# TurakhiaLab/WEPP

Hardware: AMD Instinct MI355X
Metric: reads placed/sec on SARS-CoV-2 MAT (~16M nodes) (higher is better)
Workload: dtype int32

## Files before the change

__graft_entry__.py:

```python
import os
import subprocess
import sys

ROOT = os.path.dirname(os.path.abspath(__file__))
if ROOT not in sys.path:
    sys.path.insert(0, ROOT)
sys.path.insert(0, os.path.join(ROOT, "tests"))


def build():
    subprocess.check_call(["make", "-C", os.path.join(ROOT, "wepp_amd", "csrc"), "-j4"])
    csrc = os.path.join(ROOT, "wepp_amd", "csrc")
    variant = os.path.join(ROOT, "variants", "win64", "libwepp_place.so")
    newest = max(os.path.getmtime(os.path.join(csrc, f)) for f in os.listdir(csrc) if f.endswith((".hip", ".cpp", ".hpp")))
    if not os.path.exists(variant) or os.path.getmtime(variant) < newest:
        subprocess.check_call(["bash", os.path.join(ROOT, "tools", "build_variant.sh"), "win64", "-DWEPP_WIN_SIZE=64", "-DWEPP_WIN_STRIDE=32"],
                              stdout=subprocess.DEVNULL)
    import oracle_bridge
    oracle_bridge.build()
    import wepp_amd


def smoke():
    import numpy as np
    import oracle_bridge
    import wepp_amd as w

    g = w.generate_tree(7, 3000, genome_len=2000, p_ambiguous=0.01, p_masked_node=0.002, root_mutations=2)
    reads = g.reads(8, 256, read_len=150, amplicon_len=400, amplicon_step=300, p_substitution=0.004, p_n=0.01,
                    p_iupac=0.1)
    mat = w.Mat(g.tree, device=0)
    res = mat.place_batch(reads)
    want = oracle_bridge.OracleTree(g.tree).place_batch(reads, nthreads=4)
    assert (res.score == want["score"]).all(), "parsimony scores differ from the oracle"
    assert (res.best_bfs_j == want["best_j"]).all(), "placement nodes differ from the oracle"
    assert (res.num_best == want["num_best"]).all(), "num_best differs from the oracle"
    assert (res.has_unique == want["has_unique"]).all(), "has_unique differs from the oracle"
    mat.close()
    print("smoke ok: %d reads placed on a %d-node MAT, bit-exact vs oracle" % (reads.n_reads, g.tree.n_nodes))

# ... 6 lines not shown
```

wepp_amd/csrc/capi.cpp:

```cpp
#include <hip/hip_runtime.h>

#include <algorithm>
#include <atomic>
#include <functional>
#include <cstdio>
#include <cstdlib>
#include <chrono>
#include <cstring>
#include <new>
#include <string>
#include <thread>
#include <vector>

#include "handle.hpp"
#include "host_pool.hpp"

namespace {

std::atomic<uint32_t> g_handles_alive{0};

void release(wepp_mat* h) {
    if (!h) return;
    g_handles_alive.fetch_sub(1, std::memory_order_relaxed);
    (void)hipSetDevice(h->device);
// ... 178 lines not shown
                a_nest.insert(a_nest.end(), st.ix_nest.begin(), st.ix_nest.end());
                a_nrec.insert(a_nrec.end(), st.nrec.begin(), st.nrec.end());
                a_pre.insert(a_pre.end(), st.rq_pre.begin(), st.rq_pre.end());
                a_suf.insert(a_suf.end(), st.rq_suf.begin(), st.rq_suf.end());
                a_dst.insert(a_dst.end(), st.rq_dst.begin(), st.rq_dst.end());
                a_sp.insert(a_sp.end(), st.sp.begin(), st.sp.end());
                h->wc_nodes += st.n;
                h->wc_count++;
            }
        DevWalk arena{};
        auto dev_array = [&](auto*& out, size_t count, const auto& front) -> int {
            using T = std::remove_cv_t<std::remove_reference_t<decltype(front[0])>>;
            void* p = nullptr;
            const size_t bytes = std::max<size_t>(count * sizeof(T), 16);
            hipError_t e2 = hipMalloc(&p, bytes);
            if (e2 != hipSuccess) return set_error(WEPP_ENOMEM, std::string("hipMalloc: ") + hipGetErrorString(e2));
            h->allocs.push_back(p);
            h->stats.device_bytes += bytes;
            if (!front.empty()) HIP_TRY(hipMemcpy(p, front.data(), front.size() * sizeof(T), hipMemcpyHostToDevice));
            out = (T*)p;
            return WEPP_OK;
        };
        IxHead* g_head; IxEnt* g_ent; uint8_t *g_nest, *g_sp; NodeRec* g_nrec; SegNode *g_pre, *g_suf, *g_dst;
#define ARR(ptr, count, front) if ((rc = dev_array(ptr, count, front)) != WEPP_OK) { release(h); return rc; }
        ARR(g_head, tot_head, a_head) ARR(g_ent, tot_ent, a_ent) ARR(g_nest, tot_head, a_nest) ARR(g_sp, tot_sp, a_sp)
        ARR(g_nrec, tot_n, a_nrec) ARR(g_pre, tot_n, a_pre) ARR(g_suf, tot_n, a_suf) ARR(g_dst, tot_dst, a_dst)
#undef ARR
        arena.ix_head = g_head; arena.ix_ent = g_ent; arena.ix_nest = g_nest; arena.sp = g_sp;
        arena.nrec = g_nrec; arena.rq_pre = g_pre; arena.rq_suf = g_suf; arena.rq_dst = g_dst;
        {
            size_t o_n = wc_n, o_ent = wc_ent, o_head = wc_head, o_sp = wc_sp, o_dst = wc_dst;
            for (size_t i = 0; i < f.streams.size(); i++) {
                const Stream& st = f.streams[i];
                WcInfo& wi = info[n_wc + i];
                wi.n = st.n;
                wi.rq_blocks = st.rq_blocks;
                wi.last_ent = (uint32_t)(o_ent + st.ix_ent.size() - 1);
                wi.has_pre = st.ix_pre.empty() ? 0u : st.ix_pre[0];
                wi.node_off = (uint32_t)o_n; wi.head_off = (uint32_t)o_head; wi.nest_off = (uint32_t)o_head; wi.dst_off = (uint32_t)o_dst;
                wi.sp_off = o_sp;
                wi.tau = st.tau;
                wi.whole = st.whole;
                wi.whole_bfs = f.rank2bfs[st.whole.rank < f.N ? st.whole.rank : 0u];
#define CP(dst, off, vec) if (!vec.empty()) HIP_TRY(hipMemcpy(dst + off, vec.data(), vec.size() * sizeof(vec[0]), hipMemcpyHostToDevice));
                CP(g_head, o_head, st.ix_head) CP(g_ent, o_ent, st.ix_ent) CP(g_nest, o_head, st.ix_nest) CP(g_sp, o_sp, st.sp)
                CP(g_nrec, o_n, st.nrec) CP(g_pre, o_n, st.rq_pre) CP(g_suf, o_n, st.rq_suf) CP(g_dst, o_dst, st.rq_dst)
#undef CP
                if (o_ent) HIP_TRY(launch_rebase_index(g_head + o_head, (uint32_t)st.ix_head.size(), g_ent + o_ent, (uint32_t)st.ix_ent.size(), (uint32_t)o_ent, nullptr));
                DevWalk& dw = h->walks[i];
                dw.n = st.n; dw.rq_blocks = st.rq_blocks; dw.last_ent = wi.last_ent; dw.has_pre = wi.has_pre; dw.whole = st.whole;
                dw.ix_head = g_head + o_head; dw.ix_ent = g_ent; dw.ix_nest = g_nest + o_head; dw.nrec = g_nrec + o_n;
                dw.rq_pre = g_pre + o_n; dw.rq_suf = g_suf + o_n; dw.rq_dst = g_dst + o_dst; dw.sp = g_sp + o_sp;
                o_n += st.n; o_ent += st.ix_ent.size(); o_head += st.ix_head.size(); o_sp += st.sp.size(); o_dst += st.rq_dst.size();
            }
            HIP_TRY(hipDeviceSynchronize());
        }
        d.tw_base = (uint32_t)n_wc;
        {
            std::vector<int64_t> s_nkey;
            std::vector<uint32_t> s_nstat, s_node0, s_eoff, s_evw, s_cpo, s_cpw;
            std::vector<uint8_t> s_meta, s_lb;
            std::vector<BlkSum> s_sum;
            struct Off { size_t nkey, node0, eoff, sum, ev, cpo, cpw; };
            std::vector<Off> offs;
            for (const auto& wc : f.wcrowns)
                for (const Stream& st : wc) {
                    offs.push_back(Off{s_nkey.size(), s_node0.size(), s_eoff.size(), s_sum.size(), s_evw.size(), s_cpo.size(), s_cpw.size()});
                    s_nkey.insert(s_nkey.end(), st.nkey.begin(), st.nkey.end());
                    s_nstat.insert(s_nstat.end(), st.nstat.begin(), st.nstat.end());
                    s_node0.insert(s_node0.end(), st.blk_node0.begin(), st.blk_node0.end());
                    s_eoff.insert(s_eoff.end(), st.blk_eoff.begin(), st.blk_eoff.end());
// ... 15 lines not shown
            std::vector<DevStream> ws(f.wcrowns.size() * WC_MAX, DevStream{});
            size_t k = 0;
            for (size_t w = 0; w < f.wcrowns.size(); w++)
                for (size_t i = 0; i < f.wcrowns[w].size(); i++, k++) {
                    const Stream& st = f.wcrowns[w][i];
                    DevStream& ds = ws[w * WC_MAX + i];
                    ds.n = st.n; ds.NB = st.NB; ds.cp_stride = st.cp_stride; ds.ncp = (uint32_t)st.cp_off.size() - 1;
                    ds.eager = 1u; ds.tier = WC_SLOT; ds.e_pad = (uint32_t)st.E;
                    ds.nkey = d_nkey + offs[k].nkey; ds.nstat = d_nstat + offs[k].nkey;
                    ds.blk_node0 = d_node0 + offs[k].node0; ds.blk_eoff = d_eoff + offs[k].eoff; ds.blk_sum = d_sum + offs[k].sum;
                    ds.ev_word = d_evw + offs[k].ev; ds.ev_meta = d_meta + offs[k].ev; ds.ev_lb = d_lb + offs[k].ev;
                    ds.cp_off = d_cpo + offs[k].cpo; ds.cp_word = d_cpw + offs[k].cpw;
                }
            UP(d.wc_streams, ws)
        }
        UP(d.wc_info, info)
        d.wc_windows = (uint32_t)f.wcrowns.size();
        h->stats.n_window_crowns = h->wc_count;
        h->stats.window_crown_nodes = h->wc_nodes;
        h->walks.resize(MAX_STREAMS, DevWalk{});
        h->walks[WC_SLOT] = arena;
    }
    UP(d.walks, h->walks)
    d.seed_sig = nullptr;
    d.seed_stride = d.seed_chunks = d.seed_row_words = 0;
    if (!f.seed_sig.empty()) {
        UP(d.seed_sig, f.seed_sig)
        d.seed_stride = f.seed_stride;
        d.seed_chunks = f.seed_chunks;
        d.seed_row_words = f.seed_row_words;
    }
    h->use_seeds = h->tun.seed ? 1 : 0;
    h->stats.seed_chunks = d.seed_chunks;
    h->stats.seed_chunk_blocks = d.seed_stride;
    h->stats.seed_sig_bytes = (uint64_t)f.seed_sig.size() * 4;
    h->stats.window_size = WIN_SIZE;
    h->stats.window_stride = WIN_STRIDE;
    h->stats.window_uncovered_positions = f.max_pos + 1 > MAX_WINDOWS * WIN_STRIDE ? f.max_pos + 1 - MAX_WINDOWS * WIN_STRIDE : 0;
#undef UP
    {
        const bool walk_on = h->tun.walk;
        h->walk_ok = 1;
        for (const Stream& st : f.streams)
            if ((uint64_t)st.n >= (1ull << (32 - WALK_DELTA_BITS))) h->walk_ok = 0;
        h->use_walk = (walk_on && h->walk_ok) ? 1 : 0;
    }
// ... 1398 lines not shown
```

wepp_amd/csrc/device_mat.hpp:

```cpp
#pragma once
#include <hip/hip_runtime.h>
#include <stdint.h>

#include "flatmat.hpp"

namespace wepp {

constexpr int32_t SCORE_INF_DEV = SCORE_INF;
constexpr uint32_t NS_CNT_MASK_DEV = NS_CNT_MASK;
constexpr uint32_t NS_LEAF_DEV = NS_LEAF, NS_MASKED_DEV = NS_MASKED, NS_ELIG0_DEV = NS_ELIG0, NS_ROOT_DEV = NS_ROOT;
constexpr uint32_t EV_OFF_MASK_DEV = EV_OFF_MASK;
constexpr uint32_t W_EXIT_DEV = W_EXIT, W_LEAF_DEV = W_LEAF, W_PAD_DEV = W_PAD;
constexpr uint32_t WEPP_FLAG_HAS_UNIQUE_DEV = WEPP_FLAG_HAS_UNIQUE;

constexpr uint32_t EV_TAIL_PAD = 128, SUM_TAIL_PAD = 4;
struct DevStream {
    uint32_t n, NB, cp_stride, ncp;
    uint32_t eager;
    uint32_t tier;
    uint32_t e_pad;
    const int64_t* nkey;
    const uint32_t* nstat;
    const uint32_t* blk_node0;
    const uint32_t* blk_eoff;
    const BlkSum* blk_sum;
    const uint32_t* ev_word;
    const uint8_t* ev_meta;
// ... 4 lines not shown
};

struct DevWalk {
    uint32_t n, rq_blocks, last_ent, has_pre;
    SegNode whole;
    const IxHead* ix_head;
    const IxEnt* ix_ent;
    const uint8_t* ix_nest;
    const NodeRec* nrec;
    const SegNode* rq_pre;
    const SegNode* rq_suf;
    const SegNode* rq_dst;
    const uint8_t* sp;
};

struct WcInfo {
    uint32_t n, rq_blocks, last_ent, has_pre;
    uint32_t node_off, head_off, nest_off, dst_off;
    unsigned long long sp_off;
    int32_t tau;
    uint32_t whole_bfs;
    SegNode whole;
};

struct DevMAT {
    uint32_t N, bm_words, max_pos, n_streams;
    uint32_t n_windows;
    uint32_t walk_eager_nodes;
    int32_t root_base;
    int32_t tau[MAX_STREAMS];
    const uint32_t* node_woff;
    const uint32_t* words;
    const uint32_t* nstat;
    const uint32_t* rank2dfs;
    const uint32_t* dfs2bfs;
    const uint32_t* rank2bfs;
    const uint32_t* bfs2dfs;
    const uint32_t* parent_dfs;
    const uint8_t* maxnest;
    const DevWalk* walks;
    const WcInfo* wc_info;
    const DevStream* wc_streams;
    uint32_t wc_windows;
    uint32_t tw_base;
    uint32_t win_n[MAX_WINDOWS];
    const uint32_t* seed_sig;
    uint32_t seed_stride, seed_chunks, seed_row_words;
};
constexpr uint32_t WIN_MIN_ENTRIES = 32;

constexpr uint32_t MAX_PLANS = 128;
constexpr uint32_t PLAN_WALK8 = 0, PLAN_WALK16 = 1, PLAN_SWEEP = 2, PLAN_WALKC8 = 3, PLAN_WALKC16 = 4, PLAN_WIN = 5, PLAN_SEED = 6;
constexpr uint32_t PLAN_WIN_BASE = PLAN_WIN * MAX_STREAMS;
constexpr uint32_t PLAN_SEED_ID = PLAN_WIN_BASE + MAX_WINDOWS;
static_assert(PLAN_SEED_ID < MAX_PLANS, "plan ids");
__host__ __device__ inline uint32_t plan_id(uint32_t cls, uint32_t idx) { return cls == PLAN_SEED ? PLAN_SEED_ID : cls * MAX_STREAMS + idx; }
__host__ __device__ inline uint32_t plan_class(uint32_t id) { return id == PLAN_SEED_ID ? PLAN_SEED : id >= PLAN_WIN_BASE ? PLAN_WIN : id / MAX_STREAMS; }
__host__ __device__ inline uint32_t plan_index(uint32_t id) { return id == PLAN_SEED_ID ? 0u : id >= PLAN_WIN_BASE ? id - PLAN_WIN_BASE : id % MAX_STREAMS; }
constexpr uint32_t SEED_MIN_HARD = 3;
constexpr uint32_t SEED_MIN_STREAM_NODES = 65536;
constexpr uint32_t SEED_MAX_ENTRIES = 4096;
#ifndef WEPP_SEED_THREADS
#define WEPP_SEED_THREADS 512
#endif
constexpr uint32_t SEED_THREADS = WEPP_SEED_THREADS;
constexpr uint32_t SEED_HEAVY_LEVEL_MIN = 256, SEED_HEAVY_PARTS = 32, SEED_HEAVY_CAP = 128;
constexpr uint32_t SEED_MAX_HARD = 255;
// ... 90 lines not shown
constexpr uint32_t ROUTE_BLOCKS = WEPP_ROUTE_BLOCKS;
constexpr uint32_t ROUTE_THREADS = 1024;

struct RouteDirect {
    uint32_t* wlist[2];
    uint32_t* clist[2];
    uint32_t* jobs[2];
    uint32_t* job_first;
    uint32_t* wwlist;
    uint32_t* best_bfs_j;
    int32_t* score;
    uint32_t* num_best;
    uint32_t* flags;
    unsigned long long* work_counter;
    uint32_t cand_min;
    uint32_t ww_max_small, ww_max_big;
};
hipError_t launch_route(const DevMAT& m, const uint32_t* d_read_off, const uint32_t* d_read_word, uint32_t n_reads,
                        int use_crowns, uint32_t walk_max_events, uint32_t job_events, uint32_t stack8, uint32_t stack16,
                        uint32_t seed_min_hard, uint32_t seed_min_nodes,
                        uint32_t* job_n, uint8_t* tier_of, int32_t* root_score, uint32_t* blk_counts,
                        uint32_t* tier_info, uint32_t* slot_in_blk, uint32_t* tier_info_next, uint32_t* wsid, const RouteDirect& direct,
                        hipStream_t stream);
hipError_t launch_rebase_index(IxHead* heads, uint32_t n_heads, IxEnt* ents, uint32_t n_ents, uint32_t ent_off, hipStream_t stream);
uint32_t seed_lds_bytes(const DevMAT& m, uint32_t ent_cap);
hipError_t seed_set_max_lds(uint32_t bytes);
size_t seed_heavy_bytes();
hipError_t launch_seed(const DevMAT& m, const DevStream& full, const uint32_t* list, uint32_t n_list, uint32_t ent_cap,
                       const uint32_t* d_read_off, const uint32_t* d_read_word, const int32_t* root_score,
                       uint32_t* best_bfs_j, int32_t* score, uint32_t* num_best, uint32_t* flags,
                       unsigned long long* work_counter, void* heavy_table, hipStream_t stream);
constexpr uint32_t SORT_KEY_BITS = 21;
constexpr uint32_t SORT_MIN_READS = 4096;
constexpr uint32_t WALK_SORT_KEY_BITS = SORT_KEY_BITS + 4;
constexpr uint32_t WALK_SORT_MIN_READS = 32768;
static_assert(MAX_STREAMS <= 16, "stream index in the walks' sort key");
hipError_t launch_first_pos(const uint32_t* list, uint32_t n, const uint32_t* d_read_off, const uint32_t* d_read_word,
                            uint32_t* keys, hipStream_t stream);
hipError_t launch_walk_keys(const uint32_t* list, uint32_t n, const uint8_t* tier_of, const uint32_t* d_read_off,
                            const uint32_t* d_read_word, uint32_t* keys, hipStream_t stream);
hipError_t sort_reads_temp_bytes(uint32_t n, size_t* bytes);
hipError_t launch_sort_reads(const uint32_t* keys_in, uint32_t* keys_out, const uint32_t* vals_in, uint32_t* vals_out,
                             uint32_t n, void* temp, size_t temp_bytes, hipStream_t stream, uint32_t key_bits = SORT_KEY_BITS);
hipError_t launch_scatter(const uint8_t* tier_of, const uint32_t* slot_in_blk, uint32_t n_reads, const uint32_t* blk_counts,
                          uint32_t* tier_info, uint32_t* list, bool skip_plain_walks, hipStream_t stream);
hipError_t launch_sweep(const DevMAT& m, const DevStream& st, const uint32_t* d_read_off,
// ... 85 lines not shown
```

wepp_amd/csrc/flat_debug.cpp:

```cpp
#include <cstdlib>
#include <cstring>
#include <new>
#include <string>

#include "../../include/wepp_place.h"
#include "errors.hpp"
#include "flatmat.hpp"

extern "C" uint64_t wepp_debug_flatten_count(void) { return wepp::flatten_count(); }

extern "C" int wepp_flat_create(const wepp_tree_desc* tree, wepp_flat_t** out) {
    if (!tree || !out) return wepp::set_error(WEPP_EINVAL, "null argument");
    *out = nullptr;
    wepp_flat* h = new (std::nothrow) wepp_flat();
    if (!h) return wepp::set_error(WEPP_ENOMEM, "out of host memory");
    std::string err;
    int rc;
    try {
        rc = wepp::flatten_tree(*tree, h->f, err);
    } catch (const std::bad_alloc&) {
        delete h;
        return wepp::set_error(WEPP_ENOMEM, "out of host memory while flattening the tree");
    }
    if (rc != WEPP_OK) { delete h; return wepp::set_error(rc, err); }
    *out = h;
    return WEPP_OK;
}

extern "C" int wepp_flat_get(const wepp_flat_t* flat, const char* name, const void** data, uint64_t* count,
                             uint32_t* elem_bytes) {
    if (!flat || !name || !data || !count || !elem_bytes) return wepp::set_error(WEPP_EINVAL, "null argument");
    const wepp::FlatMAT& f = flat->f;
// ... 99 lines not shown
```

wepp_amd/csrc/route_kernels.hip:

```cpp
#include <hip/hip_runtime.h>
#include <stdint.h>

#include <algorithm>

#include "device_mat.hpp"
#include "place_dev.hpp"

namespace wepp {

#ifdef WEPP_ROUTE_STATS
__device__ unsigned long long g_route_stats[16];
#define ROUTE_STAMP(i) do { __builtin_amdgcn_sched_barrier(0); __builtin_amdgcn_s_waitcnt(0); { const unsigned long long now_ = __builtin_amdgcn_s_memtime(); \
    if (blockIdx.x == 0 && threadIdx.x == 0) g_route_stats[i] += now_ - last_; last_ = now_; } __builtin_amdgcn_sched_barrier(0); } while (0)
#define ROUTE_STAMP_NW(i) do { __builtin_amdgcn_sched_barrier(0); { const unsigned long long now_ = __builtin_amdgcn_s_memtime(); \
    if (blockIdx.x == 0 && threadIdx.x == 0) g_route_stats[i] += now_ - last_; last_ = now_; } __builtin_amdgcn_sched_barrier(0); } while (0)
#else
#define ROUTE_STAMP(i)
#define ROUTE_STAMP_NW(i)
#endif

__global__ __launch_bounds__(ROUTE_THREADS) void k_route(DevMAT m, const uint32_t* __restrict__ read_off,
                                                          const uint32_t* __restrict__ read_word, uint32_t n_reads,
                                                          int use_crowns, uint32_t walk_max_events, uint32_t job_events,
                                                          uint32_t stack8, uint32_t stack16,
                                                          uint32_t seed_min_hard, uint32_t seed_min_nodes,
                                                          uint32_t* __restrict__ job_n, uint8_t* __restrict__ tier_of,
                                                          int32_t* __restrict__ root_score,
                                                          uint32_t* __restrict__ blk_counts,
                                                          uint32_t* __restrict__ tier_info,
                                                          uint32_t* __restrict__ slot_in_blk,
                                                          uint32_t* __restrict__ tier_info_next,
                                                          uint32_t* __restrict__ wsid, RouteDirect direct) {
#ifdef WEPP_ROUTE_STATS
    unsigned long long last_ = __builtin_amdgcn_s_memtime();
#endif
    __shared__ uint32_t cnt[MAX_PLANS], mx[MAX_PLANS], jobs_of[2 * MAX_STREAMS], open_of[4], events_of[2], resolved_of[1];
    constexpr uint32_t RT_MAX = MAX_WINDOWS * WC_MAX + MAX_STREAMS;
    __shared__ int32_t wc_tau[RT_MAX], rt_wbase[RT_MAX];
    __shared__ uint32_t wc_n[RT_MAX], rt_head[RT_MAX], rt_nest[RT_MAX], rt_wbfs[RT_MAX], rt_wcnt[RT_MAX];
    for (uint32_t i = threadIdx.x; i < m.tw_base + m.n_streams && i < RT_MAX; i += blockDim.x) {
        const WcInfo q = m.wc_info[i];
        wc_tau[i] = q.tau; wc_n[i] = q.n; rt_head[i] = q.head_off; rt_nest[i] = q.nest_off;
        rt_wbase[i] = q.whole.base; rt_wbfs[i] = q.whole_bfs; rt_wcnt[i] = (q.whole.cnt << 1) | (q.whole.hu ? 1u : 0u);
    }
    constexpr uint32_t TT_MAX = 64, WT_D = 8;
    __shared__ uint8_t t_tab[TT_MAX], sid_tab[MAX_WINDOWS * WT_D];
    __shared__ uint32_t tab_ok[1];
    if (threadIdx.x == 0) tab_ok[0] = (m.n_streams >= 2 && m.tau[m.n_streams - 2] < (int32_t)TT_MAX && m.tau[0] >= 0) ? 1u : 0u;
    __syncthreads();
    if (threadIdx.x < TT_MAX) {
        uint32_t t = m.n_streams - 1;
        for (uint32_t i = 0; i + 1 < m.n_streams; i++)
            if ((int32_t)threadIdx.x <= m.tau[i]) { t = i; break; }
        t_tab[threadIdx.x] = (uint8_t)t;
    }
    if (threadIdx.x < m.wc_windows * WT_D && threadIdx.x < MAX_WINDOWS * WT_D) {
        const uint32_t wi = threadIdx.x / WT_D, d = threadIdx.x % WT_D;
        uint32_t pick = 0xFFu;
        for (uint32_t i = 0; i < WC_MAX; i++) {
            const int32_t tau = wc_tau[wi * WC_MAX + i];
            if (!wc_n[wi * WC_MAX + i]) break;
            if (tau != 0x7FFFFFFF && (tau < m.root_base || tau >= m.root_base + (int32_t)(WT_D - 1))) atomicAnd(&tab_ok[0], 0u);
            if (pick == 0xFFu && m.root_base + (int32_t)d <= tau) pick = i;
        }
        sid_tab[threadIdx.x] = (uint8_t)pick;
    }
    __shared__ uint32_t wl_count[2], wl_base[2], cj_count[2], cl_count[2], cj_base[2], cl_base[2], c_ok[2], ww_count[2], ww_base[2], w16_to_wave[1], ww_cand[2];
    if (threadIdx.x < 2) { cj_count[threadIdx.x] = 0; cl_count[threadIdx.x] = 0; }
    if (threadIdx.x == 0) ww_count[0] = ww_count[1] = ww_cand[0] = ww_cand[1] = 0;
    if (threadIdx.x == 0) resolved_of[0] = 0;
    if (threadIdx.x < 2) wl_count[threadIdx.x] = 0;
    if (blockIdx.x == 0 && threadIdx.x < TI_WORDS) tier_info_next[threadIdx.x] = 0;
    if (threadIdx.x < MAX_PLANS) { cnt[threadIdx.x] = 0; mx[threadIdx.x] = 0; }
    if (threadIdx.x < 4) open_of[threadIdx.x] = 0;
    if (threadIdx.x < 2) events_of[threadIdx.x] = 0;
    if (threadIdx.x < 2 * MAX_STREAMS) jobs_of[threadIdx.x] = 0;
    __syncthreads();
    ROUTE_STAMP(0);
    const uint32_t per = (n_reads + gridDim.x - 1) / gridDim.x;
    const uint32_t lo = blockIdx.x * per, hi = min(n_reads, lo + per);
    const IxHead* __restrict__ ar_head = m.walks[WC_SLOT].ix_head;
    const uint8_t* __restrict__ ar_nest = m.walks[WC_SLOT].ix_nest;
    const uint32_t root_w0 = m.node_woff[0], root_w1 = m.node_woff[1];
    const bool use_tabs = tab_ok[0] != 0;
    const uint32_t lane = threadIdx.x & 63;
    const unsigned long long lt_mask = (1ull << lane) - 1ull;
    for (uint32_t rbase = lo; rbase < hi; rbase += 4 * blockDim.x) {
      const uint32_t r0 = rbase + threadIdx.x;
      uint32_t so4[4], k4[4], fw[4][2];
      uint32_t app4[4] = {0, 0, 0, 0}, aslot4[4] = {0, 0, 0, 0};
      uint32_t cj4[4] = {0, 0, 0, 0}, cjs4[4] = {0, 0, 0, 0}, cls4[4] = {0, 0, 0, 0}, cnj4[4] = {0, 0, 0, 0};
      uint32_t ww4[4] = {0, 0, 0, 0};
#pragma unroll
      for (uint32_t u = 0; u < 4; u++) {
          const uint32_t r = r0 + u * blockDim.x;
          so4[u] = r < hi ? read_off[r] : 0u;
          k4[u] = r < hi ? read_off[r + 1] - so4[u] : 0u;
      }
#pragma unroll
      for (uint32_t u = 0; u < 4; u++)
#pragma unroll
          for (uint32_t j = 0; j < 2; j++) fw[u][j] = k4[u] > j ? read_word[so4[u] + j] : 0u;
      ROUTE_STAMP(1);
      int c4[4] = {0, 0, 0, 0};
      uint32_t nh4[4] = {0, 0, 0, 0}, t4[4] = {0, 0, 0, 0}, sid4[4] = {NONE, NONE, NONE, NONE}, wi4[4] = {0, 0, 0, 0}, inwin4[4] = {0, 0, 0, 0};
      uint32_t pre_nest[4][2] = {{0, 0}, {0, 0}, {0, 0}, {0, 0}}, pre_o0[4][2] = {{0, 0}, {0, 0}, {0, 0}, {0, 0}}, pre_o1[4][2] = {{0, 0}, {0, 0}, {0, 0}, {0, 0}};
#pragma unroll
      for (uint32_t u = 0; u < 4; u++) {
        const uint32_t r = r0 + u * blockDim.x;
        const uint32_t k = k4[u], so = so4[u];
        if (r < hi) {
            int c = 0;
            auto count = [&](uint32_t sw) { if (!rw_missing(sw)) c += ((rw_mut(sw) & rw_ref(sw)) == 0) ? 1 : 0; };
            if (k > 0) count(fw[u][0]);
            if (k > 1) count(fw[u][1]);
            for (uint32_t j = 2; j < k; j++) count(read_word[so + j]);
            nh4[u] = (uint32_t)c;
            for (uint32_t w = root_w0; w < root_w1; w++) {
                const uint32_t tw = m.words[w];
                uint32_t sw = NONE;
                if (k <= 2) {
                    if (k > 0 && w_pos(fw[u][0]) == w_pos(tw)) sw = fw[u][0];
                    if (k > 1 && w_pos(fw[u][1]) == w_pos(tw)) sw = fw[u][1];
                } else sw = find_entry(read_word, so, k, w_pos(tw));
                if (sw != NONE) c += enter_delta(tw, sw);
            }
            c4[u] = c;
            ROUTE_STAMP_NW(2);
            const int theta = m.root_base + c + (int)k;
// ... 10 lines not shown
                const uint32_t p_lo = w_pos(fw[u][0]), p_hi = w_pos(k > 2 ? read_word[so + k - 1] : k == 2 ? fw[u][1] : fw[u][0]);
                const uint32_t wi = p_lo / WIN_STRIDE;
                wi4[u] = wi;
                inwin4[u] = p_hi < wi * WIN_STRIDE + WIN_SIZE ? 1u : 0u;
                if (inwin4[u] && wi < m.wc_windows) {
                    const int rs = m.root_base + c;
                    if (use_tabs) {
                        const uint32_t i = sid_tab[wi * WT_D + (uint32_t)min(max(c, 0), (int)WT_D - 1)];
                        if (i != 0xFFu && wc_n[wi * WC_MAX + i] < wc_n[m.tw_base + t]) sid4[u] = wi * WC_MAX + i;
                    } else
                        for (uint32_t i = 0; i < WC_MAX; i++) {
                            const uint32_t qn = wc_n[wi * WC_MAX + i];
                            if (!qn) break;
                            if (rs <= wc_tau[wi * WC_MAX + i]) { if (qn < wc_n[m.tw_base + t]) sid4[u] = wi * WC_MAX + i; break; }
                        }
                }
            }
            ROUTE_STAMP_NW(4);
            if (walk_max_events && k <= WALK16_K) {
                const uint32_t tab = sid4[u] != NONE ? sid4[u] : m.tw_base + t;
#pragma unroll
                for (uint32_t j = 0; j < 2; j++) {
                    const uint32_t p = w_pos(fw[u][j]);
                    if (j < k && p <= m.max_pos) {
                        pre_nest[u][j] = (uint32_t)ar_nest[rt_nest[tab] + p];
                        pre_o0[u][j] = ar_head[rt_head[tab] + p].off;
                        pre_o1[u][j] = ar_head[rt_head[tab] + p + 1].off;
                    }
                }
            }
        }
      }
      ROUTE_STAMP(5);
#pragma unroll
      for (uint32_t u = 0; u < 4; u++) {
        const uint32_t r = r0 + u * blockDim.x;
        const bool valid = r < hi;
        uint32_t t_id = 0, append = 0;
        bool resolved = false;
        const uint32_t k = k4[u];
        if (valid) {
        const uint32_t so = so4[u];
        const int c = c4[u];
        const uint32_t n_hard = nh4[u];
        uint32_t t = t4[u];
        const uint32_t sid = sid4[u], wi = wi4[u];
        const bool in_win = inwin4[u] != 0;
        const uint32_t pre_tab = sid != NONE ? sid : m.tw_base + t;
        uint32_t cls = PLAN_SWEEP;
        auto classify = [&](uint32_t tab, uint32_t& nj_out, uint32_t& open_out, uint32_t& ev_out) -> uint32_t {
            const IxHead* ix_head = ar_head + rt_head[tab];
            const uint8_t* ix_nest = ar_nest + rt_nest[tab];
            uint32_t open_max = 0, events = 0, longest = 0;
            for (uint32_t j = 0; j < k; j++) {
                const uint32_t p = w_pos(j == 0 ? fw[u][0] : j == 1 ? fw[u][1] : read_word[so + j]);
                if (p <= m.max_pos) {
                    uint32_t nest, o0, o1;
                    if (j < 2 && tab == pre_tab) { nest = j ? pre_nest[u][1] : pre_nest[u][0]; o0 = j ? pre_o0[u][1] : pre_o0[u][0]; o1 = j ? pre_o1[u][1] : pre_o1[u][0]; }
                    else { nest = (uint32_t)ix_nest[p]; o0 = ix_head[p].off; o1 = ix_head[p + 1].off; }
                    open_max += nest;
                    const uint32_t len = o1 - o0 - 1u;
                    events += len;
                    longest = max(longest, len);
                }
            }
            open_out = open_max;
            ev_out = events;
            nj_out = 0;
            if (events <= walk_max_events) {
                if (k <= WALK8_K && open_max <= stack8) return PLAN_WALK8;
                if (open_max <= stack16) return PLAN_WALK16;
                return PLAN_SWEEP;
            }
            if (open_max > stack16) return PLAN_SWEEP;
            const uint32_t small = (k <= WALK8_K && open_max <= stack8) ? 1u : 0u;
            const uint32_t je = small ? (job_events & 0xFFFFu) : (job_events >> 16);
            nj_out = min((events + je - 1) / je, longest);
            return small ? PLAN_WALKC8 : PLAN_WALKC16;
        };
        if (walk_max_events && k <= WALK16_K) {
            uint32_t nj = 0, open_max = 0, events = 0;
            if (sid != NONE) {
                cls = classify(sid, nj, open_max, events);
                if (cls != PLAN_SWEEP) { wsid[r] = sid; t = WC_SLOT; }
// ... 74 lines not shown
            }
            if (listed) slot_in_blk[r] = slot;
        }
        {
            const unsigned long long rm = __ballot(resolved);
            if (rm && lane == (uint32_t)__builtin_ctzll(rm)) atomicAdd(&resolved_of[0], (uint32_t)__popcll(rm));
        }
        if (direct.wlist[0]) {
#pragma unroll
            for (uint32_t cc = 0; cc < 2; cc++) {
                const unsigned long long mk = __ballot(append == cc + 1);
                if (!mk) continue;
                const int first = __builtin_ctzll(mk);
                uint32_t base = 0;
                if ((int)lane == first) base = atomicAdd(&wl_count[cc], (uint32_t)__popcll(mk));
                base = (uint32_t)__builtin_amdgcn_readlane((int)base, first);
                if (append == cc + 1) { app4[u] = cc + 1; aslot4[u] = base + (uint32_t)__popcll(mk & lt_mask); }
            }
        }
        ROUTE_STAMP(6);
      }
      if (direct.wlist[0]) {
          __syncthreads();
          if (threadIdx.x < 2) {
              const uint32_t cc = threadIdx.x;
              const bool to_wave = cc == 1 && direct.wwlist && wl_count[1] && wl_count[1] <= WALK16_TO_WAVE_MAX;
              if (cc == 1) w16_to_wave[0] = to_wave ? 1u : 0u;
              if (to_wave) {
                  wl_base[1] = atomicAdd(&tier_info[TI_WWCUR], wl_count[1]);
                  atomicAdd(&tier_info[TI_W16WAVE], wl_count[1]);
              } else
                  wl_base[cc] = wl_count[cc] ? atomicAdd(&tier_info[TI_WCUR + cc], wl_count[cc]) : 0u;
              wl_count[cc] = 0;
              c_ok[cc] = 0;
              if (cl_count[cc] && direct.jobs[0]) {
                  cj_base[cc] = atomicAdd(&tier_info[TI_JCUR + cc], cj_count[cc]);
                  cl_base[cc] = atomicAdd(&tier_info[TI_CCUR + cc], cl_count[cc]);
                  if (cj_base[cc] + cj_count[cc] > BLIND_JOB_CAP || cl_base[cc] + cl_count[cc] > BLIND_CHUNKED_READS) tier_info[TI_JOVER + cc] = 1u;
                  else c_ok[cc] = 1;
              }
              cj_count[cc] = 0;
              cl_count[cc] = 0;
              if (cc == 0) {
                  for (uint32_t b = 0; b < 2; b++) {
                      const uint32_t n = min(ww_count[b], b ? direct.ww_max_big : direct.ww_max_small);
                      ww_base[b] = n ? atomicAdd(&tier_info[TI_WWCUR + b], n) : 0u;
                      ww_count[b] = 0;
                  }
              }
          }
          __syncthreads();
#pragma unroll
          for (uint32_t u = 0; u < 4; u++) {
              const uint32_t r = r0 + u * blockDim.x;
              if (app4[u]) (app4[u] == 1 ? direct.wlist[0] : w16_to_wave[0] ? direct.wwlist : direct.wlist[1])[wl_base[app4[u] - 1] + aslot4[u]] = r;
              if (ww4[u]) {
                  const uint32_t big = ww4[u] & 1u, at = ww_base[big] + (ww4[u] >> 1) - 1u;
                  direct.wwlist[big ? n_reads - 1u - at : at] = r;
              }
              if (cj4[u] && c_ok[cj4[u] - 1]) {
                  const uint32_t cc = cj4[u] - 1, j0 = cj_base[cc] + cjs4[u];
                  (cc ? direct.clist[1] : direct.clist[0])[cl_base[cc] + cls4[u]] = r;
                  direct.job_first[r] = j0;
                  uint32_t* jt = cc ? direct.jobs[1] : direct.jobs[0];
                  for (uint32_t c2 = 0; c2 < cnj4[u]; c2++) jt[j0 + c2] = r;
              }
          }
          __syncthreads();
      }
      ROUTE_STAMP(7);
    }
    __syncthreads();
// ... 9 lines not shown
    if (threadIdx.x < 2 && events_of[threadIdx.x]) atomicAdd(&tier_info[TI_EVENTS + threadIdx.x], (events_of[threadIdx.x] + 63) >> 6);
    if (threadIdx.x < 2 && ww_cand[threadIdx.x]) atomicAdd(&tier_info[TI_WWCAND + threadIdx.x], ww_cand[threadIdx.x]);
    if (threadIdx.x == 0 && resolved_of[0]) {
        atomicAdd(&tier_info[TI_RESOLVED], resolved_of[0]);
        if (direct.work_counter) atomicAdd(direct.work_counter + WALK_COUNTERS + (blockIdx.x & (WALK_COUNTERS - 1)), 48ull * resolved_of[0]);
    }
    ROUTE_STAMP(8);
#ifdef WEPP_ROUTE_STATS
    if (blockIdx.x == 0 && threadIdx.x == 0) g_route_stats[9] += 1;
#endif
}
#ifdef WEPP_ROUTE_STATS
extern "C" int wepp_debug_route_stats(unsigned long long* out16) {
    return (int)hipMemcpyFromSymbol(out16, HIP_SYMBOL(g_route_stats), sizeof(g_route_stats));
}
#endif

__global__ void k_rebase_index(IxHead* __restrict__ heads, uint32_t n_heads, IxEnt* __restrict__ ents, uint32_t n_ents, uint32_t ent_off) {
    const uint32_t i = blockIdx.x * blockDim.x + threadIdx.x;
    if (i < n_heads) heads[i].off += ent_off;
    if (i < n_ents && ents[i].up != IX_NONE) ents[i].up += ent_off;
}

__global__ __launch_bounds__(ROUTE_THREADS) void k_scatter(const uint8_t* __restrict__ tier_of,
                                                            const uint32_t* __restrict__ slot_in_blk, uint32_t n_reads,
                                                            const uint32_t* __restrict__ blk_counts,
                                                            uint32_t* __restrict__ tier_info,
                                                            uint32_t* __restrict__ list, int skip_plain_walks) {
    __shared__ uint32_t base[MAX_PLANS], before[MAX_PLANS];
    if (threadIdx.x < MAX_PLANS) before[threadIdx.x] = 0;
    __syncthreads();
    {
        const uint32_t t = threadIdx.x & (MAX_PLANS - 1), c0 = threadIdx.x / MAX_PLANS;
        uint32_t acc = 0;
        for (uint32_t b = c0; b < blockIdx.x; b += blockDim.x / MAX_PLANS) acc += blk_counts[b * MAX_PLANS + t];
        if (acc) atomicAdd(&before[t], acc);
    }
    __syncthreads();
    if (threadIdx.x < MAX_PLANS) {
        const uint32_t t = threadIdx.x;
        uint32_t off = 0;
        for (uint32_t i = 0; i < t; i++) off += tier_info[TI_COUNT + i];
        base[t] = off + before[t];
        if (blockIdx.x == 0) {
            tier_info[TI_OFF + t] = off;
            if (t == MAX_PLANS - 1) tier_info[TI_OFF + MAX_PLANS] = off + tier_info[TI_COUNT + t];
// ... 28 lines not shown
}

__global__ void k_walk_keys(const uint32_t* __restrict__ list, uint32_t n, const uint8_t* __restrict__ tier_of,
                            const uint32_t* __restrict__ read_off, const uint32_t* __restrict__ read_word,
                            uint32_t* __restrict__ keys) {
    const uint32_t i = blockIdx.x * blockDim.x + threadIdx.x;
    if (i >= n) return;
    const uint32_t r = list[i], so = read_off[r];
    const uint32_t first = (read_off[r + 1] > so) ? w_pos(read_word[so]) + 1u : 0u;
    keys[i] = (plan_index(tier_of[r]) << SORT_KEY_BITS) | first;
}

hipError_t launch_route(const DevMAT& m, const uint32_t* d_read_off, const uint32_t* d_read_word, uint32_t n_reads,
                        int use_crowns, uint32_t walk_max_events, uint32_t job_events, uint32_t stack8, uint32_t stack16,
                        uint32_t seed_min_hard, uint32_t seed_min_nodes, uint32_t* job_n, uint8_t* tier_of,
                        int32_t* root_score, uint32_t* blk_counts, uint32_t* tier_info, uint32_t* slot_in_blk,
                        uint32_t* tier_info_next, uint32_t* wsid, const RouteDirect& direct, hipStream_t stream) {
    hipLaunchKernelGGL(k_route, dim3(ROUTE_BLOCKS), dim3(ROUTE_THREADS), 0, stream, m, d_read_off, d_read_word,
                       n_reads, use_crowns, walk_max_events, job_events, std::min(stack8, WALK8_STACK), std::min(stack16, WALK16_STACK),
                       seed_min_hard, seed_min_nodes, job_n, tier_of, root_score, blk_counts, tier_info, slot_in_blk, tier_info_next, wsid, direct);
    return hipGetLastError();
}

hipError_t launch_rebase_index(IxHead* heads, uint32_t n_heads, IxEnt* ents, uint32_t n_ents, uint32_t ent_off, hipStream_t stream) {
    const uint32_t n = std::max(n_heads, n_ents);
    if (!n) return hipSuccess;
    hipLaunchKernelGGL(k_rebase_index, dim3((n + 255) / 256), dim3(256), 0, stream, heads, n_heads, ents, n_ents, ent_off);
    return hipGetLastError();
}

hipError_t launch_first_pos(const uint32_t* list, uint32_t n, const uint32_t* d_read_off, const uint32_t* d_read_word,
                            uint32_t* keys, hipStream_t stream) {
    if (n == 0) return hipSuccess;
    hipLaunchKernelGGL(k_first_pos, dim3((n + 255) / 256), dim3(256), 0, stream, list, n, d_read_off, d_read_word, keys);
    return hipGetLastError();
}

hipError_t launch_walk_keys(const uint32_t* list, uint32_t n, const uint8_t* tier_of, const uint32_t* d_read_off,
                            const uint32_t* d_read_word, uint32_t* keys, hipStream_t stream) {
    if (n == 0) return hipSuccess;
    hipLaunchKernelGGL(k_walk_keys, dim3((n + 255) / 256), dim3(256), 0, stream, list, n, tier_of, d_read_off, d_read_word, keys);
    return hipGetLastError();
}

hipError_t launch_scatter(const uint8_t* tier_of, const uint32_t* slot_in_blk, uint32_t n_reads, const uint32_t* blk_counts,
                          uint32_t* tier_info, uint32_t* list, bool skip_plain_walks, hipStream_t stream) {
    hipLaunchKernelGGL(k_scatter, dim3(ROUTE_BLOCKS), dim3(ROUTE_THREADS), 0, stream, tier_of, slot_in_blk, n_reads,
                       blk_counts, tier_info, list, skip_plain_walks ? 1 : 0);
    return hipGetLastError();
}

}
```

Baseline: 10.91 billion.

## Precompute packed per-position route words and route tables once at load

Adds a load-time pass that packs each index position's event-list length and nesting depth into one dword, so the route classifier does one load per position instead of a byte plus two IxHead offsets. The per-block shared-memory routing tables, previously rebuilt at the start of every k_route block, are now built once by a one-block kernel and bulk-copied into LDS. The end-of-batch atomic reservations are also spread across a wave's lanes instead of being serialized in two threads. It costs an extra device array the size of the index heads and falls back to the old two-offset path when a length saturates.

```diff
diff --git a/__graft_entry__.py b/__graft_entry__.py
--- a/__graft_entry__.py
+++ b/__graft_entry__.py
@@ -11,11 +11,11 @@
 def build():
     subprocess.check_call(["make", "-C", os.path.join(ROOT, "wepp_amd", "csrc"), "-j4"])
     csrc = os.path.join(ROOT, "wepp_amd", "csrc")
-    variant = os.path.join(ROOT, "variants", "win64", "libwepp_place.so")
     newest = max(os.path.getmtime(os.path.join(csrc, f)) for f in os.listdir(csrc) if f.endswith((".hip", ".cpp", ".hpp")))
-    if not os.path.exists(variant) or os.path.getmtime(variant) < newest:
-        subprocess.check_call(["bash", os.path.join(ROOT, "tools", "build_variant.sh"), "win64", "-DWEPP_WIN_SIZE=64", "-DWEPP_WIN_STRIDE=32"],
-                              stdout=subprocess.DEVNULL)
+    for name, flags in (("win64", ["-DWEPP_WIN_SIZE=64", "-DWEPP_WIN_STRIDE=32"]), ("rtlen3", ["-DWEPP_RT_LEN_BITS=3"])):
+        variant = os.path.join(ROOT, "variants", name, "libwepp_place.so")
+        if not os.path.exists(variant) or os.path.getmtime(variant) < newest:
+            subprocess.check_call(["bash", os.path.join(ROOT, "tools", "build_variant.sh"), name, *flags], stdout=subprocess.DEVNULL)
     import oracle_bridge
     oracle_bridge.build()
     import wepp_amd
diff --git a/wepp_amd/csrc/capi.cpp b/wepp_amd/csrc/capi.cpp
--- a/wepp_amd/csrc/capi.cpp
+++ b/wepp_amd/csrc/capi.cpp
@@ -224,12 +224,20 @@
             return WEPP_OK;
         };
         IxHead* g_head; IxEnt* g_ent; uint8_t *g_nest, *g_sp; NodeRec* g_nrec; SegNode *g_pre, *g_suf, *g_dst;
+        uint32_t* g_rtpos;
 #define ARR(ptr, count, front) if ((rc = dev_array(ptr, count, front)) != WEPP_OK) { release(h); return rc; }
         ARR(g_head, tot_head, a_head) ARR(g_ent, tot_ent, a_ent) ARR(g_nest, tot_head, a_nest) ARR(g_sp, tot_sp, a_sp)
         ARR(g_nrec, tot_n, a_nrec) ARR(g_pre, tot_n, a_pre) ARR(g_suf, tot_n, a_suf) ARR(g_dst, tot_dst, a_dst)
+        ARR(g_rtpos, tot_head, std::vector<uint32_t>())
 #undef ARR
         arena.ix_head = g_head; arena.ix_ent = g_ent; arena.ix_nest = g_nest; arena.sp = g_sp;
         arena.nrec = g_nrec; arena.rq_pre = g_pre; arena.rq_suf = g_suf; arena.rq_dst = g_dst;
+        d.rt_pos = g_rtpos;
+        for (size_t w = 0; w < f.wcrowns.size(); w++)
+            for (size_t i = 0; i < f.wcrowns[w].size(); i++) {
+                const WcInfo& wi = info[w * WC_MAX + i];
+                HIP_TRY(launch_route_pos(g_head + wi.head_off, g_nest + wi.nest_off, (uint32_t)f.wcrowns[w][i].ix_head.size(), g_rtpos + wi.head_off, nullptr));
+            }
         {
             size_t o_n = wc_n, o_ent = wc_ent, o_head = wc_head, o_sp = wc_sp, o_dst = wc_dst;
             for (size_t i = 0; i < f.streams.size(); i++) {
@@ -249,6 +257,7 @@
                 CP(g_nrec, o_n, st.nrec) CP(g_pre, o_n, st.rq_pre) CP(g_suf, o_n, st.rq_suf) CP(g_dst, o_dst, st.rq_dst)
 #undef CP
                 if (o_ent) HIP_TRY(launch_rebase_index(g_head + o_head, (uint32_t)st.ix_head.size(), g_ent + o_ent, (uint32_t)st.ix_ent.size(), (uint32_t)o_ent, nullptr));
+                HIP_TRY(launch_route_pos(g_head + o_head, g_nest + o_head, (uint32_t)st.ix_head.size(), g_rtpos + o_head, nullptr));
                 DevWalk& dw = h->walks[i];
                 dw.n = st.n; dw.rq_blocks = st.rq_blocks; dw.last_ent = wi.last_ent; dw.has_pre = wi.has_pre; dw.whole = st.whole;
                 dw.ix_head = g_head + o_head; dw.ix_ent = g_ent; dw.ix_nest = g_nest + o_head; dw.nrec = g_nrec + o_n;
@@ -310,6 +319,12 @@
         h->walks[WC_SLOT] = arena;
     }
     UP(d.walks, h->walks)
+    {
+        const std::vector<RouteTables> blank(1);
+        UP(d.route_tab, blank)
+        HIP_TRY(launch_route_tables(d, const_cast<RouteTables*>(d.route_tab), nullptr));
+        HIP_TRY(hipDeviceSynchronize());
+    }
     d.seed_sig = nullptr;
     d.seed_stride = d.seed_chunks = d.seed_row_words = 0;
     if (!f.seed_sig.empty()) {
diff --git a/wepp_amd/csrc/device_mat.hpp b/wepp_amd/csrc/device_mat.hpp
--- a/wepp_amd/csrc/device_mat.hpp
+++ b/wepp_amd/csrc/device_mat.hpp
@@ -3,6 +3,7 @@
 #include <stdint.h>
 
 #include "flatmat.hpp"
+#include "route_pos.hpp"
 
 namespace wepp {
 
@@ -53,6 +54,16 @@
     uint32_t whole_bfs;
     SegNode whole;
 };
+
+constexpr uint32_t RT_MAX = MAX_WINDOWS * WC_MAX + MAX_STREAMS;
+constexpr uint32_t RT_TT_MAX = 64, RT_WT_D = 8;
+struct RouteTables {
+    int32_t wc_tau[RT_MAX], rt_wbase[RT_MAX];
+    uint32_t wc_n[RT_MAX], rt_head[RT_MAX], rt_wbfs[RT_MAX], rt_wcnt[RT_MAX];
+    uint32_t tab_ok;
+    uint8_t t_tab[RT_TT_MAX], sid_tab[MAX_WINDOWS * RT_WT_D];
+};
+static_assert(sizeof(RouteTables) % 4 == 0, "copied dword by dword");
 
 struct DevMAT {
     uint32_t N, bm_words, max_pos, n_streams;
@@ -74,6 +85,8 @@
     const DevStream* wc_streams;
     uint32_t wc_windows;
     uint32_t tw_base;
+    const RouteTables* route_tab;
+    const uint32_t* rt_pos;
     uint32_t win_n[MAX_WINDOWS];
     const uint32_t* seed_sig;
     uint32_t seed_stride, seed_chunks, seed_row_words;
@@ -210,6 +223,8 @@
                         uint32_t* job_n, uint8_t* tier_of, int32_t* root_score, uint32_t* blk_counts,
                         uint32_t* tier_info, uint32_t* slot_in_blk, uint32_t* tier_info_next, uint32_t* wsid, const RouteDirect& direct,
                         hipStream_t stream);
+hipError_t launch_route_tables(const DevMAT& m, RouteTables* out, hipStream_t stream);
+hipError_t launch_route_pos(const IxHead* heads, const uint8_t* nest, uint32_t n_heads, uint32_t* out, hipStream_t stream);
 hipError_t launch_rebase_index(IxHead* heads, uint32_t n_heads, IxEnt* ents, uint32_t n_ents, uint32_t ent_off, hipStream_t stream);
 uint32_t seed_lds_bytes(const DevMAT& m, uint32_t ent_cap);
 hipError_t seed_set_max_lds(uint32_t bytes);
diff --git a/wepp_amd/csrc/flat_debug.cpp b/wepp_amd/csrc/flat_debug.cpp
--- a/wepp_amd/csrc/flat_debug.cpp
+++ b/wepp_amd/csrc/flat_debug.cpp
@@ -6,8 +6,10 @@
 #include "../../include/wepp_place.h"
 #include "errors.hpp"
 #include "flatmat.hpp"
+#include "route_pos.hpp"
 
 extern "C" uint64_t wepp_debug_flatten_count(void) { return wepp::flatten_count(); }
+extern "C" uint32_t wepp_debug_route_len_bits(void) { return wepp::RT_LEN_BITS; }
 
 extern "C" int wepp_flat_create(const wepp_tree_desc* tree, wepp_flat_t** out) {
     if (!tree || !out) return wepp::set_error(WEPP_EINVAL, "null argument");
diff --git a/wepp_amd/csrc/route_kernels.hip b/wepp_amd/csrc/route_kernels.hip
--- a/wepp_amd/csrc/route_kernels.hip
+++ b/wepp_amd/csrc/route_kernels.hip
@@ -18,6 +18,38 @@
 #define ROUTE_STAMP(i)
 #define ROUTE_STAMP_NW(i)
 #endif
+
+__global__ __launch_bounds__(ROUTE_THREADS) void k_route_tables(DevMAT m, RouteTables* __restrict__ out) {
+    __shared__ RouteTables rt;
+    for (uint32_t i = threadIdx.x; i < sizeof(RouteTables) / 4; i += blockDim.x) ((uint32_t*)&rt)[i] = 0u;
+    __syncthreads();
+    for (uint32_t i = threadIdx.x; i < m.tw_base + m.n_streams && i < RT_MAX; i += blockDim.x) {
+        const WcInfo q = m.wc_info[i];
+        rt.wc_tau[i] = q.tau; rt.wc_n[i] = q.n; rt.rt_head[i] = q.head_off;
+        rt.rt_wbase[i] = q.whole.base; rt.rt_wbfs[i] = q.whole_bfs; rt.rt_wcnt[i] = (q.whole.cnt << 1) | (q.whole.hu ? 1u : 0u);
+    }
+    if (threadIdx.x == 0) rt.tab_ok = (m.n_streams >= 2 && m.tau[m.n_streams - 2] < (int32_t)RT_TT_MAX && m.tau[0] >= 0) ? 1u : 0u;
+    __syncthreads();
+    if (threadIdx.x < RT_TT_MAX) {
+        uint32_t t = m.n_streams - 1;
+        for (uint32_t i = 0; i + 1 < m.n_streams; i++)
+            if ((int32_t)threadIdx.x <= m.tau[i]) { t = i; break; }
+        rt.t_tab[threadIdx.x] = (uint8_t)t;
+    }
+    if (threadIdx.x < m.wc_windows * RT_WT_D && threadIdx.x < MAX_WINDOWS * RT_WT_D) {
+        const uint32_t wi = threadIdx.x / RT_WT_D, d = threadIdx.x % RT_WT_D;
+        uint32_t pick = 0xFFu;
+        for (uint32_t i = 0; i < WC_MAX; i++) {
+            const int32_t tau = rt.wc_tau[wi * WC_MAX + i];
+            if (!rt.wc_n[wi * WC_MAX + i]) break;
+            if (tau != 0x7FFFFFFF && (tau < m.root_base || tau >= m.root_base + (int32_t)(RT_WT_D - 1))) atomicAnd(&rt.tab_ok, 0u);
+            if (pick == 0xFFu && m.root_base + (int32_t)d <= tau) pick = i;
+        }
+        rt.sid_tab[threadIdx.x] = (uint8_t)pick;
+    }
+    __syncthreads();
+    for (uint32_t i = threadIdx.x; i < sizeof(RouteTables) / 4; i += blockDim.x) ((uint32_t*)out)[i] = ((const uint32_t*)&rt)[i];
+}
 
 __global__ __launch_bounds__(ROUTE_THREADS) void k_route(DevMAT m, const uint32_t* __restrict__ read_off,
                                                           const uint32_t* __restrict__ read_word, uint32_t n_reads,
@@ -35,36 +67,12 @@
     unsigned long long last_ = __builtin_amdgcn_s_memtime();
 #endif
     __shared__ uint32_t cnt[MAX_PLANS], mx[MAX_PLANS], jobs_of[2 * MAX_STREAMS], open_of[4], events_of[2], resolved_of[1];
-    constexpr uint32_t RT_MAX = MAX_WINDOWS * WC_MAX + MAX_STREAMS;
-    __shared__ int32_t wc_tau[RT_MAX], rt_wbase[RT_MAX];
-    __shared__ uint32_t wc_n[RT_MAX], rt_head[RT_MAX], rt_nest[RT_MAX], rt_wbfs[RT_MAX], rt_wcnt[RT_MAX];
-    for (uint32_t i = threadIdx.x; i < m.tw_base + m.n_streams && i < RT_MAX; i += blockDim.x) {
-        const WcInfo q = m.wc_info[i];
-        wc_tau[i] = q.tau; wc_n[i] = q.n; rt_head[i] = q.head_off; rt_nest[i] = q.nest_off;
-        rt_wbase[i] = q.whole.base; rt_wbfs[i] = q.whole_bfs; rt_wcnt[i] = (q.whole.cnt << 1) | (q.whole.hu ? 1u : 0u);
-    }
-    constexpr uint32_t TT_MAX = 64, WT_D = 8;
-    __shared__ uint8_t t_tab[TT_MAX], sid_tab[MAX_WINDOWS * WT_D];
-    __shared__ uint32_t tab_ok[1];
-    if (threadIdx.x == 0) tab_ok[0] = (m.n_streams >= 2 && m.tau[m.n_streams - 2] < (int32_t)TT_MAX && m.tau[0] >= 0) ? 1u : 0u;
-    __syncthreads();
-    if (threadIdx.x < TT_MAX) {
-        uint32_t t = m.n_streams - 1;
-        for (uint32_t i = 0; i + 1 < m.n_streams; i++)
-            if ((int32_t)threadIdx.x <= m.tau[i]) { t = i; break; }
-        t_tab[threadIdx.x] = (uint8_t)t;
-    }
-    if (threadIdx.x < m.wc_windows * WT_D && threadIdx.x < MAX_WINDOWS * WT_D) {
-        const uint32_t wi = threadIdx.x / WT_D, d = threadIdx.x % WT_D;
-        uint32_t pick = 0xFFu;
-        for (uint32_t i = 0; i < WC_MAX; i++) {
-            const int32_t tau = wc_tau[wi * WC_MAX + i];
-            if (!wc_n[wi * WC_MAX + i]) break;
-            if (tau != 0x7FFFFFFF && (tau < m.root_base || tau >= m.root_base + (int32_t)(WT_D - 1))) atomicAnd(&tab_ok[0], 0u);
-            if (pick == 0xFFu && m.root_base + (int32_t)d <= tau) pick = i;
-        }
-        sid_tab[threadIdx.x] = (uint8_t)pick;
-    }
+    __shared__ RouteTables rt;
+    for (uint32_t i = threadIdx.x; i < sizeof(RouteTables) / 4; i += blockDim.x) ((uint32_t*)&rt)[i] = ((const uint32_t*)m.route_tab)[i];
+    constexpr uint32_t TT_MAX = RT_TT_MAX, WT_D = RT_WT_D;
+    const auto& wc_tau = rt.wc_tau; const auto& rt_wbase = rt.rt_wbase; const auto& wc_n = rt.wc_n; const auto& rt_head = rt.rt_head;
+    const auto& rt_wbfs = rt.rt_wbfs; const auto& rt_wcnt = rt.rt_wcnt;
+    const auto& t_tab = rt.t_tab; const auto& sid_tab = rt.sid_tab;
     __shared__ uint32_t wl_count[2], wl_base[2], cj_count[2], cl_count[2], cj_base[2], cl_base[2], c_ok[2], ww_count[2], ww_base[2], w16_to_wave[1], ww_cand[2];
     if (threadIdx.x < 2) { cj_count[threadIdx.x] = 0; cl_count[threadIdx.x] = 0; }
     if (threadIdx.x == 0) ww_count[0] = ww_count[1] = ww_cand[0] = ww_cand[1] = 0;
@@ -79,10 +87,9 @@
     ROUTE_STAMP(0);
     const uint32_t per = (n_reads + gridDim.x - 1) / gridDim.x;
     const uint32_t lo = blockIdx.x * per, hi = min(n_reads, lo + per);
-    const IxHead* __restrict__ ar_head = m.walks[WC_SLOT].ix_head;
-    const uint8_t* __restrict__ ar_nest = m.walks[WC_SLOT].ix_nest;
+    const uint32_t* __restrict__ ar_pos = m.rt_pos;
     const uint32_t root_w0 = m.node_woff[0], root_w1 = m.node_woff[1];
-    const bool use_tabs = tab_ok[0] != 0;
+    const bool use_tabs = rt.tab_ok != 0;
     const uint32_t lane = threadIdx.x & 63;
     const unsigned long long lt_mask = (1ull << lane) - 1ull;
     for (uint32_t rbase = lo; rbase < hi; rbase += 4 * blockDim.x) {
@@ -104,7 +111,7 @@
       ROUTE_STAMP(1);
       int c4[4] = {0, 0, 0, 0};
       uint32_t nh4[4] = {0, 0, 0, 0}, t4[4] = {0, 0, 0, 0}, sid4[4] = {NONE, NONE, NONE, NONE}, wi4[4] = {0, 0, 0, 0}, inwin4[4] = {0, 0, 0, 0};
-      uint32_t pre_nest[4][2] = {{0, 0}, {0, 0}, {0, 0}, {0, 0}}, pre_o0[4][2] = {{0, 0}, {0, 0}, {0, 0}, {0, 0}}, pre_o1[4][2] = {{0, 0}, {0, 0}, {0, 0}, {0, 0}};
+      uint32_t pre_w[4][2] = {{0, 0}, {0, 0}, {0, 0}, {0, 0}};
 #pragma unroll
       for (uint32_t u = 0; u < 4; u++) {
         const uint32_t r = r0 + u * blockDim.x;
@@ -161,11 +168,7 @@
 #pragma unroll
                 for (uint32_t j = 0; j < 2; j++) {
                     const uint32_t p = w_pos(fw[u][j]);
-                    if (j < k && p <= m.max_pos) {
-                        pre_nest[u][j] = (uint32_t)ar_nest[rt_nest[tab] + p];
-                        pre_o0[u][j] = ar_head[rt_head[tab] + p].off;
-                        pre_o1[u][j] = ar_head[rt_head[tab] + p + 1].off;
-                    }
+                    if (j < k && p <= m.max_pos) pre_w[u][j] = ar_pos[rt_head[tab] + p];
                 }
             }
         }
@@ -188,17 +191,17 @@
         const uint32_t pre_tab = sid != NONE ? sid : m.tw_base + t;
         uint32_t cls = PLAN_SWEEP;
         auto classify = [&](uint32_t tab, uint32_t& nj_out, uint32_t& open_out, uint32_t& ev_out) -> uint32_t {
-            const IxHead* ix_head = ar_head + rt_head[tab];
-            const uint8_t* ix_nest = ar_nest + rt_nest[tab];
+            const uint32_t* ix_pos = ar_pos + rt_head[tab];
             uint32_t open_max = 0, events = 0, longest = 0;
             for (uint32_t j = 0; j < k; j++) {
                 const uint32_t p = w_pos(j == 0 ? fw[u][0] : j == 1 ? fw[u][1] : read_word[so + j]);
                 if (p <= m.max_pos) {
-                    uint32_t nest, o0, o1;
-                    if (j < 2 && tab == pre_tab) { nest = j ? pre_nest[u][1] : pre_nest[u][0]; o0 = j ? pre_o0[u][1] : pre_o0[u][0]; o1 = j ? pre_o1[u][1] : pre_o1[u][0]; }
-                    else { nest = (uint32_t)ix_nest[p]; o0 = ix_head[p].off; o1 = ix_head[p + 1].off; }
+                    uint32_t nest, len;
+                    if (!rt_pos_unpack(j < 2 && tab == pre_tab ? (j ? pre_w[u][1] : pre_w[u][0]) : ix_pos[p], len, nest)) {
+                        const IxHead* ix_head = m.walks[WC_SLOT].ix_head + rt_head[tab];
+                        len = ix_head[p + 1].off - ix_head[p].off - 1u;
+                    }
                     open_max += nest;
-                    const uint32_t len = o1 - o0 - 1u;
                     events += len;
                     longest = max(longest, len);
                 }
@@ -319,32 +322,29 @@
       }
       if (direct.wlist[0]) {
           __syncthreads();
-          if (threadIdx.x < 2) {
-              const uint32_t cc = threadIdx.x;
-              const bool to_wave = cc == 1 && direct.wwlist && wl_count[1] && wl_count[1] <= WALK16_TO_WAVE_MAX;
-              if (cc == 1) w16_to_wave[0] = to_wave ? 1u : 0u;
-              if (to_wave) {
-                  wl_base[1] = atomicAdd(&tier_info[TI_WWCUR], wl_count[1]);
-                  atomicAdd(&tier_info[TI_W16WAVE], wl_count[1]);
-              } else
-                  wl_base[cc] = wl_count[cc] ? atomicAdd(&tier_info[TI_WCUR + cc], wl_count[cc]) : 0u;
-              wl_count[cc] = 0;
-              c_ok[cc] = 0;
-              if (cl_count[cc] && direct.jobs[0]) {
-                  cj_base[cc] = atomicAdd(&tier_info[TI_JCUR + cc], cj_count[cc]);
-                  cl_base[cc] = atomicAdd(&tier_info[TI_CCUR + cc], cl_count[cc]);
-                  if (cj_base[cc] + cj_count[cc] > BLIND_JOB_CAP || cl_base[cc] + cl_count[cc] > BLIND_CHUNKED_READS) tier_info[TI_JOVER + cc] = 1u;
-                  else c_ok[cc] = 1;
+          if (threadIdx.x < 64) {
+              const uint32_t l = threadIdx.x, cc = l & 1u;
+              const bool to_wave = direct.wwlist && wl_count[1] && wl_count[1] <= WALK16_TO_WAVE_MAX;
+              const bool chunked = l >= 4 && l < 8 && cl_count[cc] && direct.jobs[0];
+              uint32_t n = 0, word = 0;
+              if (l < 2) { n = wl_count[l]; word = (l == 1 && to_wave) ? TI_WWCUR : TI_WCUR + l; }
+              else if (l < 4) { n = min(ww_count[cc], cc ? direct.ww_max_big : direct.ww_max_small); word = TI_WWCUR + cc; }
+              else if (chunked) { n = l < 6 ? cj_count[cc] : cl_count[cc]; word = (l < 6 ? TI_JCUR : TI_CCUR) + cc; }
+              uint32_t base = 0;
+              if (n) base = atomicAdd(&tier_info[word], n);
+              if (l == 1 && to_wave) atomicAdd(&tier_info[TI_W16WAVE], n);
+              const uint32_t peer = (uint32_t)__shfl((int)base, (int)(l ^ 2u));
+              if (l < 2) wl_base[l] = base;
+              else if (l < 4) ww_base[cc] = base;
+              else if (l < 6) {
+                  cj_base[cc] = base;
+                  cl_base[cc] = peer;
+                  const bool over = chunked && (base + n > BLIND_JOB_CAP || peer + cl_count[cc] > BLIND_CHUNKED_READS);
+                  if (over) tier_info[TI_JOVER + cc] = 1u;
+                  c_ok[cc] = chunked && !over ? 1u : 0u;
               }
-              cj_count[cc] = 0;
-              cl_count[cc] = 0;
-              if (cc == 0) {
-                  for (uint32_t b = 0; b < 2; b++) {
-                      const uint32_t n = min(ww_count[b], b ? direct.ww_max_big : direct.ww_max_small);
-                      ww_base[b] = n ? atomicAdd(&tier_info[TI_WWCUR + b], n) : 0u;
-                      ww_count[b] = 0;
-                  }
-              }
+              if (l == 1) w16_to_wave[0] = to_wave ? 1u : 0u;
+              if (l < 2) { wl_count[l] = 0; ww_count[l] = 0; cj_count[l] = 0; cl_count[l] = 0; }
           }
           __syncthreads();
 #pragma unroll
@@ -400,6 +400,12 @@
     if (i < n_ents && ents[i].up != IX_NONE) ents[i].up += ent_off;
 }
 
+__global__ void k_route_pos(const IxHead* __restrict__ heads, const uint8_t* __restrict__ nest, uint32_t n_heads, uint32_t* __restrict__ out) {
+    const uint32_t i = blockIdx.x * blockDim.x + threadIdx.x;
+    if (i >= n_heads) return;
+    out[i] = i + 1 < n_heads ? rt_pos_pack(heads[i + 1].off - heads[i].off - 1u, nest[i]) : 0u;
+}
+
 __global__ __launch_bounds__(ROUTE_THREADS) void k_scatter(const uint8_t* __restrict__ tier_of,
                                                             const uint32_t* __restrict__ slot_in_blk, uint32_t n_reads,
                                                             const uint32_t* __restrict__ blk_counts,
@@ -474,6 +480,11 @@
     return hipGetLastError();
 }
 
+hipError_t launch_route_tables(const DevMAT& m, RouteTables* out, hipStream_t stream) {
+    hipLaunchKernelGGL(k_route_tables, dim3(1), dim3(ROUTE_THREADS), 0, stream, m, out);
+    return hipGetLastError();
+}
+
 hipError_t launch_rebase_index(IxHead* heads, uint32_t n_heads, IxEnt* ents, uint32_t n_ents, uint32_t ent_off, hipStream_t stream) {
     const uint32_t n = std::max(n_heads, n_ents);
     if (!n) return hipSuccess;
@@ -481,6 +492,12 @@
     return hipGetLastError();
 }
 
+hipError_t launch_route_pos(const IxHead* heads, const uint8_t* nest, uint32_t n_heads, uint32_t* out, hipStream_t stream) {
+    if (!n_heads) return hipSuccess;
+    hipLaunchKernelGGL(k_route_pos, dim3((n_heads + 255) / 256), dim3(256), 0, stream, heads, nest, n_heads, out);
+    return hipGetLastError();
+}
+
 hipError_t launch_first_pos(const uint32_t* list, uint32_t n, const uint32_t* d_read_off, const uint32_t* d_read_word,
                             uint32_t* keys, hipStream_t stream) {
     if (n == 0) return hipSuccess;
diff --git a/wepp_amd/csrc/route_pos.hpp b/wepp_amd/csrc/route_pos.hpp
--- /dev/null
+++ b/wepp_amd/csrc/route_pos.hpp
@@ -0,0 +1,28 @@
+#pragma once
+#include <stdint.h>
+
+#ifdef __HIPCC__
+#define WEPP_RT_HD __host__ __device__
+#else
+#define WEPP_RT_HD
+#endif
+
+namespace wepp {
+
+#ifndef WEPP_RT_LEN_BITS
+#define WEPP_RT_LEN_BITS 24
+#endif
+constexpr uint32_t RT_LEN_BITS = WEPP_RT_LEN_BITS;
+static_assert(RT_LEN_BITS >= 1 && RT_LEN_BITS <= 24, "length and a byte of nesting depth share a dword");
+constexpr uint32_t RT_LEN_SAT = (1u << RT_LEN_BITS) - 1u;
+
+WEPP_RT_HD inline uint32_t rt_pos_pack(uint32_t len, uint32_t nest) {
+    return (len < RT_LEN_SAT ? len : RT_LEN_SAT) | ((nest & 0xFFu) << RT_LEN_BITS);
+}
+WEPP_RT_HD inline bool rt_pos_unpack(uint32_t word, uint32_t& len, uint32_t& nest) {
+    len = word & RT_LEN_SAT;
+    nest = (word >> RT_LEN_BITS) & 0xFFu;
+    return len != RT_LEN_SAT;
+}
+
+}
```

Result: faster. 11.57 billion (median of 6 runs) (+6.1%).
